# freewym/espresso

Measured on AMD Instinct MI355X. Metric: audio-hours/sec training (LibriSpeech Conformer-12 + CTC), higher is better.
Workload: dtype bf16; 1 GPU; LibriSpeech 960h Conformer-12 + CTC update step, <=26000 frames & <=24 utts per GPU, V=5004, on-GPU fbank+CMVN+SpecAugment, dropout 0.1, clip 2.0, Adam; parallelism=dp1

## Files before the change

### espresso_amd/csrc/flash_relpos.hip

```cpp
#include "flash_internal.h"

namespace {

typedef short bf16x4_t __attribute__((ext_vector_type(4)));
typedef const __attribute__((address_space(1))) void* gptr_t;
typedef __attribute__((address_space(3))) void* lptr_t;
typedef __attribute__((address_space(3))) bf16x4_t* lds_b4_t;

constexpr int DH = 64, TQ = 64, TK = 64;
constexpr int IMG = 64 * 128;
constexpr int BDP = 18;
constexpr int BNC = 80 * BDP * 4;
constexpr int OBP = 88;
constexpr int PP_OFF = 4 * IMG, BNC_OFF = 7 * IMG;
constexpr int LDS_BYTES = 7 * IMG + 4 * BNC;
constexpr int AUX_OFF = LDS_BYTES;
constexpr int LDS_BYTES_KV = LDS_BYTES + 1024;
constexpr float LOG2E = 1.4426950408889634f;

__device__ __forceinline__ int swz(int r) { return ((r >> 2) & 1) | (((r >> 1) & 1) << 1) | ((((r >> 2) ^ (r >> 3)) & 1) << 2); }

__device__ __forceinline__ int xcd_remap(int id, int total) {
  const int xcd = id & 7, q = total >> 3, r = total & 7;
  return (xcd < r ? xcd * (q + 1) : r * (q + 1) + (xcd - r) * q) + (id >> 3);
}
__device__ __forceinline__ f32x4_t mfma32(bf16x8_t a, bf16x8_t b, f32x4_t c) {
  return __builtin_amdgcn_mfma_f32_16x16x32_bf16(__builtin_bit_cast(__attribute__((ext_vector_type(8))) __bf16, a),
                                                 __builtin_bit_cast(__attribute__((ext_vector_type(8))) __bf16, b), c, 0, 0, 0);
}
__device__ __forceinline__ f32x4_t mfma16(bf16x4_t a, bf16x4_t b, f32x4_t c) {
  return __builtin_amdgcn_mfma_f32_16x16x16bf16_1k(a, b, c, 0, 0, 0);
}
__device__ __forceinline__ bf16x8_t cat(bf16x4_t lo, bf16x4_t hi) { return __builtin_shufflevector(lo, hi, 0, 1, 2, 3, 4, 5, 6, 7); }
__device__ __forceinline__ bf16x4_t pack4(float a, float b, float c, float d) {
  uint2 pk;
  pk.x = pack_bf2(a, b);
  pk.y = pack_bf2(c, d);
  return __builtin_bit_cast(bf16x4_t, pk);
}
__device__ __forceinline__ uint32_t lds_addr(const void* p) { return (uint32_t)(uintptr_t)p; }
template <int O0, int O1, int O2, int O3>
__device__ __forceinline__ void trr16(const uint32_t (&ad)[4], uint2 (&o)[16]) {
  asm volatile(
      "ds_read_b64_tr_b16 %0, %16 offset:%20\n\tds_read_b64_tr_b16 %1, %16 offset:%21\n\t"
      "ds_read_b64_tr_b16 %2, %16 offset:%22\n\tds_read_b64_tr_b16 %3, %16 offset:%23\n\t"
      "ds_read_b64_tr_b16 %4, %17 offset:%20\n\tds_read_b64_tr_b16 %5, %17 offset:%21\n\t"
      "ds_read_b64_tr_b16 %6, %17 offset:%22\n\tds_read_b64_tr_b16 %7, %17 offset:%23\n\t"
      "ds_read_b64_tr_b16 %8, %18 offset:%20\n\tds_read_b64_tr_b16 %9, %18 offset:%21\n\t"
      "ds_read_b64_tr_b16 %10, %18 offset:%22\n\tds_read_b64_tr_b16 %11, %18 offset:%23\n\t"
      "ds_read_b64_tr_b16 %12, %19 offset:%20\n\tds_read_b64_tr_b16 %13, %19 offset:%21\n\t"
      "ds_read_b64_tr_b16 %14, %19 offset:%22\n\tds_read_b64_tr_b16 %15, %19 offset:%23\n\t"
      "s_waitcnt lgkmcnt(0)"
      : "=&v"(o[0]), "=&v"(o[1]), "=&v"(o[2]), "=&v"(o[3]), "=&v"(o[4]), "=&v"(o[5]), "=&v"(o[6]), "=&v"(o[7]), "=&v"(o[8]),
        "=&v"(o[9]), "=&v"(o[10]), "=&v"(o[11]), "=&v"(o[12]), "=&v"(o[13]), "=&v"(o[14]), "=&v"(o[15])
      : "v"(ad[0]), "v"(ad[1]), "v"(ad[2]), "v"(ad[3]), "i"(O0), "i"(O1), "i"(O2), "i"(O3)
      : "memory");
}
template <int O0, int O1, int O2, int O3>
__device__ __forceinline__ void trr8(const uint32_t (&ad)[2], uint2 (&o)[8]) {
  asm volatile(
      "ds_read_b64_tr_b16 %0, %8 offset:%10\n\tds_read_b64_tr_b16 %1, %8 offset:%11\n\t"
      "ds_read_b64_tr_b16 %2, %8 offset:%12\n\tds_read_b64_tr_b16 %3, %8 offset:%13\n\t"
      "ds_read_b64_tr_b16 %4, %9 offset:%10\n\tds_read_b64_tr_b16 %5, %9 offset:%11\n\t"
      "ds_read_b64_tr_b16 %6, %9 offset:%12\n\tds_read_b64_tr_b16 %7, %9 offset:%13\n\t"
      "s_waitcnt lgkmcnt(0)"
      : "=&v"(o[0]), "=&v"(o[1]), "=&v"(o[2]), "=&v"(o[3]), "=&v"(o[4]), "=&v"(o[5]), "=&v"(o[6]), "=&v"(o[7])
      : "v"(ad[0]), "v"(ad[1]), "i"(O0), "i"(O1), "i"(O2), "i"(O3)
      : "memory");
}
__device__ __forceinline__ void trr20(const uint32_t (&ad)[20], uint2 (&o)[20]) {
  asm volatile(
      "ds_read_b64_tr_b16 %0, %20\n\tds_read_b64_tr_b16 %1, %21\n\tds_read_b64_tr_b16 %2, %22\n\tds_read_b64_tr_b16 %3, %23\n\t"
      "ds_read_b64_tr_b16 %4, %24\n\tds_read_b64_tr_b16 %5, %25\n\tds_read_b64_tr_b16 %6, %26\n\tds_read_b64_tr_b16 %7, %27\n\t"
      "ds_read_b64_tr_b16 %8, %28\n\tds_read_b64_tr_b16 %9, %29\n\tds_read_b64_tr_b16 %10, %30\n\tds_read_b64_tr_b16 %11, %31\n\t"
      "ds_read_b64_tr_b16 %12, %32\n\tds_read_b64_tr_b16 %13, %33\n\tds_read_b64_tr_b16 %14, %34\n\tds_read_b64_tr_b16 %15, %35\n\t"
      "ds_read_b64_tr_b16 %16, %36\n\tds_read_b64_tr_b16 %17, %37\n\tds_read_b64_tr_b16 %18, %38\n\tds_read_b64_tr_b16 %19, %39\n\t"
      "s_waitcnt lgkmcnt(0)"
      : "=&v"(o[0]), "=&v"(o[1]), "=&v"(o[2]), "=&v"(o[3]), "=&v"(o[4]), "=&v"(o[5]), "=&v"(o[6]), "=&v"(o[7]), "=&v"(o[8]),
        "=&v"(o[9]), "=&v"(o[10]), "=&v"(o[11]), "=&v"(o[12]), "=&v"(o[13]), "=&v"(o[14]), "=&v"(o[15]), "=&v"(o[16]),
        "=&v"(o[17]), "=&v"(o[18]), "=&v"(o[19])
      : "v"(ad[0]), "v"(ad[1]), "v"(ad[2]), "v"(ad[3]), "v"(ad[4]), "v"(ad[5]), "v"(ad[6]), "v"(ad[7]), "v"(ad[8]), "v"(ad[9]),
        "v"(ad[10]), "v"(ad[11]), "v"(ad[12]), "v"(ad[13]), "v"(ad[14]), "v"(ad[15]), "v"(ad[16]), "v"(ad[17]), "v"(ad[18]),
        "v"(ad[19])
      : "memory");
}
__device__ __forceinline__ uint2 lds_u2(const char* p) {
  const float* f = reinterpret_cast<const float*>(p);
  return make_uint2(__float_as_uint(f[0]), __float_as_uint(f[1]));
}
__device__ __forceinline__ bf16x8_t cat2(uint2 lo, uint2 hi) {
  return __builtin_bit_cast(bf16x8_t, make_uint4(lo.x, lo.y, hi.x, hi.y));
}
__device__ __forceinline__ void tr_image(const char* img, const uint32_t (&tro)[4], bf16x8_t (&f)[8]) {
  const uint32_t b = lds_addr(img);
  const uint32_t ad[4] = {b + tro[0], b + tro[1], b + tro[2], b + tro[3]};
  uint2 o[16];
  trr16<0, 2048, 4096, 6144>(ad, o);
#pragma unroll
  for (int dt = 0; dt < 4; ++dt) {
    f[dt * 2 + 0] = cat2(o[dt * 4 + 0], o[dt * 4 + 1]);
// ... 216 lines not shown
#pragma unroll
        for (int r = 0; r < 4; ++r)
          if (j0 + jt * 16 + g4 * 4 + r >= kl) acc_s[jt][r] = -INFINITY;
    }
    float tmax = fmaxf(fmaxf(acc_s[0][0], acc_s[0][1]), fmaxf(acc_s[0][2], acc_s[0][3]));
#pragma unroll
    for (int jt = 1; jt < 4; ++jt) tmax = fmaxf(tmax, fmaxf(fmaxf(acc_s[jt][0], acc_s[jt][1]), fmaxf(acc_s[jt][2], acc_s[jt][3])));
    tmax = fmaxf(tmax, __shfl_xor(tmax, 16, 64));
    tmax = fmaxf(tmax, __shfl_xor(tmax, 32, 64));
    const float m_new = fmaxf(m_run, tmax);
    const float msc = (m_new == -INFINITY) ? 0.f : m_new * LOG2E;
    const float alpha = fexp2(m_run * LOG2E - msc);
    float psum = 0.f;
#pragma unroll
    for (int jt = 0; jt < 4; ++jt)
#pragma unroll
      for (int r = 0; r < 4; ++r) {
        const float p = fexp2(fmaf(acc_s[jt][r], LOG2E, -msc));
        psum += p;
        acc_s[jt][r] = DROP ? fand(p, keep_mask(piece, ksh + jt * 4 + r)) : p;
      }
    l_run = l_run * alpha + psum;
    m_run = m_new;
#pragma unroll
    for (int dt = 0; dt < 4; ++dt)
#pragma unroll
      for (int r = 0; r < 4; ++r) acc_o[dt][r] *= alpha;

    {
      bf16x8_t vf[8];
      tr_image(sV, L.tro, vf);
#pragma unroll
      for (int kb = 0; kb < 2; ++kb) {
        const bf16x8_t pb = cat(pack4(acc_s[2 * kb][0], acc_s[2 * kb][1], acc_s[2 * kb][2], acc_s[2 * kb][3]),
                                pack4(acc_s[2 * kb + 1][0], acc_s[2 * kb + 1][1], acc_s[2 * kb + 1][2], acc_s[2 * kb + 1][3]));
#pragma unroll
        for (int dt = 0; dt < 4; ++dt) acc_o[dt] = mfma32(vf[dt * 2 + kb], pb, acc_o[dt]);
      }
    }
    slot_lo = slot_hi;
  }

  l_run += __shfl_xor(l_run, 16, 64);
  l_run += __shfl_xor(l_run, 32, 64);
  if (i < T) {
    const float inv = (DROP ? a.inv_keep : 1.f) / l_run;
    bf16_t* o = a.out + ((long)b * T + i) * a.ldo + h * DH;
#pragma unroll
    for (int dt = 0; dt < 4; ++dt) {
      uint2 pk;
      pk.x = pack_bf2(acc_o[dt][0] * inv, acc_o[dt][1] * inv);
      pk.y = pack_bf2(acc_o[dt][2] * inv, acc_o[dt][3] * inv);
      *reinterpret_cast<uint2*>(o + dt * 16 + g4 * 4) = pk;
    }
    if (a.lse && g4 == 0) a.lse[(long)z * T + i] = m_run + __logf(l_run);
  }
}

template <bool DROP, bool WANT_PD>
__device__ __forceinline__ void softmax_bwd_tile(f32x4_t (&acc_s)[4], const f32x4_t (&acc_dp)[4], bf16x4_t (&dsb)[4], bf16x4_t (&pdb)[4],
                                                 float lse2, float Di, float inv_keep, uint32_t piece, int ksh, int jrel_end, int g4) {
#pragma unroll
  for (int jt = 0; jt < 4; ++jt) {
    float ds[4], pd[4];
#pragma unroll
    for (int r = 0; r < 4; ++r) {
      float p = fexp2(fmaf(acc_s[jt][r], LOG2E, -lse2));
      if (jrel_end < 64 && jt * 16 + g4 * 4 + r >= jrel_end) p = 0.f;
      float dp = acc_dp[jt][r];
      if (DROP) {
        const uint32_t m = keep_mask(piece, ksh + jt * 4 + r);
        dp = fand(dp * inv_keep, m);
        if (WANT_PD) pd[r] = fand(p * inv_keep, m);
      } else if (WANT_PD) {
        pd[r] = p;
      }
      ds[r] = p * (dp - Di);
    }
    dsb[jt] = pack4(ds[0], ds[1], ds[2], ds[3]);
    if (WANT_PD) pdb[jt] = pack4(pd[0], pd[1], pd[2], pd[3]);
  }
}

template <bool DROP>
__global__ __launch_bounds__(256, 2) void rp_bwd_q_kernel(const FlashBwdArgs a) {
  __shared__ __attribute__((aligned(16))) char lds[LDS_BYTES];
  const LaneK L = lane_consts();
  const int lane = L.lane, w = L.w, li = L.li, g4 = L.g4;
  const int vid = xcd_remap(blockIdx.x, gridDim.x);
  const int z = vid / a.nq, qt = vid % a.nq;
  const int h = z / a.B, b = z % a.B;
  const int T = a.T;
  const int i0 = qt * TQ;
  const int i = i0 + 16 * w + li;
  const int kl = a.klen ? min(a.klen[b], T) : T;
  const int nt = (kl + TK - 1) / TK;
  const int nkt = (T + TK - 1) / TK;

  bf16x8_t qu[2], qv[2], dO[2];
  float Di = 0.f;
  {
    const int ic = min(i, T - 1);
    const long oq = ((long)b * T + ic) * a.ldq + h * DH + g4 * 8;
    const long oo = ((long)b * T + ic) * a.ldo + h * DH + g4 * 8;
#pragma unroll
    for (int ks = 0; ks < 2; ++ks) {
      qu[ks] = __builtin_bit_cast(bf16x8_t, *reinterpret_cast<const uint4*>(a.qu + oq + ks * 32));
      qv[ks] = __builtin_bit_cast(bf16x8_t, *reinterpret_cast<const uint4*>(a.qv + oq + ks * 32));
      const uint4 g = *reinterpret_cast<const uint4*>(a.dout + oo + ks * 32);
      const uint4 o = *reinterpret_cast<const uint4*>(a.out + oo + ks * 32);
      dO[ks] = __builtin_bit_cast(bf16x8_t, g);
      const uint32_t wg[4] = {g.x, g.y, g.z, g.w}, wo[4] = {o.x, o.y, o.z, o.w};
#pragma unroll
      for (int e = 0; e < 4; ++e)
        Di += __uint_as_float(wg[e] << 16) * __uint_as_float(wo[e] << 16) +
              __uint_as_float(wg[e] & 0xffff0000u) * __uint_as_float(wo[e] & 0xffff0000u);
    }
  }
  Di += __shfl_xor(Di, 16, 64);
  Di += __shfl_xor(Di, 32, 64);
  const float lse2 = (i < T) ? a.lse[(long)z * T + i] * LOG2E : INFINITY;
  if (i < T && g4 == 0 && a.D) a.D[(long)z * T + i] = Di;

  f32x4_t acc_t1[4], acc_t2[4];
#pragma unroll
  for (int dt = 0; dt < 4; ++dt) {
    acc_t1[dt] = (f32x4_t){0.f, 0.f, 0.f, 0.f};
    acc_t2[dt] = (f32x4_t){0.f, 0.f, 0.f, 0.f};
  }
  const bf16_t* Kb = a.k + (long)b * T * a.ldkv + h * DH;
  const bf16_t* Vb = a.v + (long)b * T * a.ldkv + h * DH;
  const bf16_t* PPb = a.pp + h * DH;
  const int R = 2 * T - 1;
  const ImgSrc srcK = img_src(Kb, a.ldkv, T - 1, w, lane), srcV = img_src(Vb, a.ldkv, T - 1, w, lane);
  const ImgSrc srcP = img_src(PPb, a.ldpp, R - 1, w, lane);
  const int pbase = (T - 1) - (i0 + TQ - 1);
  float* bd = reinterpret_cast<float*>(lds + BNC_OFF + w * BNC);
  bf16_t* ob = reinterpret_cast<bf16_t*>(bd);
  const uint32_t* bitp = DROP ? reinterpret_cast<const uint32_t*>(a.bits) + (((long)z * nkt) * (nkt * 64) + i) * 2 + (g4 >> 1) : nullptr;
  const long bit_step = (long)nkt * 64 * 2;
  const int ksh = (g4 & 1) * 16;
  uint2 mlo, mhi;
  {
    uint32_t m[4], n[4];
#pragma unroll
    for (int e = 0; e < 4; ++e) {
      m[e] = (4 * g4 + e >= 15 - li) ? 0xffffu : 0u;
      n[e] = (64 + 4 * g4 + e <= 78 - li) ? 0xffffu : 0u;
    }
    mlo = make_uint2(m[0] | (m[1] << 16), m[2] | (m[3] << 16));
    mhi = make_uint2(n[0] | (n[1] << 16), n[2] | (n[3] << 16));
  }
  const int ob_w = li * (OBP - 1) + 15 + g4 * 4;
  const char* ob_rd = reinterpret_cast<const char*>(ob) + li * (OBP * 2) + g4 * 8;

  uint32_t piece = 0, piece_next = 0;
  int jcov = 0;
  uint32_t dbd_pk[8];
  int dbd_j0 = -1;
  auto store_dbd = [&]() {
    const int j = dbd_j0 + lane;
    if (dbd_j0 >= 0 && j < T) {
      const int row_w = i0 + 16 * w, nrow = T - row_w;
      bf16_t* dp = a.dBD + ((long)z * T + row_w) * a.ld_bd + (T - 1 - row_w) + j;
      if (nrow >= 16) {
#pragma unroll
        for (int iw = 0; iw < 16; ++iw) dp[(long)iw * (a.ld_bd - 1)] = (bf16_t)(dbd_pk[iw >> 1] >> (16 * (iw & 1)));
      } else {
#pragma unroll
        for (int iw = 0; iw < 16; ++iw)
          if (iw < nrow) dp[(long)iw * (a.ld_bd - 1)] = (bf16_t)(dbd_pk[iw >> 1] >> (16 * (iw & 1)));
      }
    }
  };
  if (nt > 0) {
    issue_img(lds, srcK, 0, w, lane);
    issue_img(lds + IMG, srcV, 0, w, lane);
    issue_img(lds + PP_OFF, srcP, pbase, w, lane);
    issue_img(lds + PP_OFF + IMG, srcP, pbase + 64, w, lane);
    if (DROP) piece_next = bitp[0];
  }
  int slot_lo = 0;
  for (int t = 0; t < nt; ++t) {
    const int j0 = t * TK;
    jcov = min(T, j0 + TK);
    asm volatile("s_waitcnt vmcnt(0)" ::: "memory");
    __builtin_amdgcn_s_barrier();
    store_dbd();
    const int slot_hi = slot_lo == 2 ? 0 : slot_lo + 1;
    const int slot_nx = slot_hi == 2 ? 0 : slot_hi + 1;
    if (DROP) {
      piece = piece_next;
      asm volatile("" : "+v"(piece));
    }
    if (t + 1 < nt) {
      if (DROP) piece_next = bitp[(long)(t + 1) * bit_step];
      char* st = lds + ((t + 1) & 1) * 2 * IMG;
      issue_img(st, srcK, j0 + TK, w, lane);
      issue_img(st + IMG, srcV, j0 + TK, w, lane);
      issue_img(lds + PP_OFF + slot_nx * IMG, srcP, pbase + 64 * (t + 2), w, lane);
    }
    const char* sK = lds + (t & 1) * 2 * IMG;
    const char* sV = sK + IMG;
// ... 55 lines not shown
      for (int q16 = 0; q16 < 5; ++q16) {
        const int qq = q16 - w + 3;
        const uint32_t pbk = lds_addr(((qq >> 2) ? blk_hi : blk_lo) + (qq & 3) * 2048);
#pragma unroll
        for (int dt = 0; dt < 4; ++dt) ad[q16 * 4 + dt] = pbk + L.tro[dt];
      }
      trr20(ad, pf);
#pragma unroll
      for (int cb = 0; cb < 2; ++cb) {
        uint2 blo = lds_u2(ob_rd + cb * 64);
        const uint2 bhi = lds_u2(ob_rd + cb * 64 + 32);
        if (cb == 0) {
          blo.x &= mlo.x;
          blo.y &= mlo.y;
        }
        const bf16x8_t db = cat2(blo, bhi);
#pragma unroll
        for (int dt = 0; dt < 4; ++dt) acc_t2[dt] = mfma32(cat2(pf[(2 * cb) * 4 + dt], pf[(2 * cb + 1) * 4 + dt]), db, acc_t2[dt]);
      }
      uint2 bl = lds_u2(ob_rd + 128);
      bl.x &= mhi.x;
      bl.y &= mhi.y;
#pragma unroll
      for (int dt = 0; dt < 4; ++dt)
        acc_t2[dt] = mfma16(__builtin_bit_cast(bf16x4_t, pf[16 + dt]), __builtin_bit_cast(bf16x4_t, bl), acc_t2[dt]);
    }
    {
      const bf16_t* bs = ob + 15 + lane;
#pragma unroll
      for (int k = 0; k < 8; ++k)
        dbd_pk[k] = (uint32_t)bs[(2 * k) * (OBP - 1)] | ((uint32_t)bs[(2 * k + 1) * (OBP - 1)] << 16);
      dbd_j0 = j0;
    }
    wave_lds_sync();
    slot_lo = slot_hi;
  }
  store_dbd();

  if (i < T) {
    bf16_t* o1 = a.t1 + ((long)b * T + i) * a.ldt + h * DH;
    bf16_t* o2 = a.t2 + ((long)b * T + i) * a.ldt + h * DH;
#pragma unroll
    for (int dt = 0; dt < 4; ++dt) {
      uint2 pk;
      pk.x = pack_bf2(acc_t1[dt][0] * a.scaling, acc_t1[dt][1] * a.scaling);
      pk.y = pack_bf2(acc_t1[dt][2] * a.scaling, acc_t1[dt][3] * a.scaling);
      *reinterpret_cast<uint2*>(o1 + dt * 16 + g4 * 4) = pk;
      pk.x = pack_bf2(acc_t2[dt][0] * a.scaling, acc_t2[dt][1] * a.scaling);
      pk.y = pack_bf2(acc_t2[dt][2] * a.scaling, acc_t2[dt][3] * a.scaling);
      *reinterpret_cast<uint2*>(o2 + dt * 16 + g4 * 4) = pk;
    }
    if (a.dq) {
      bf16_t* oq = a.dq + ((long)b * T + i) * a.lddq + h * DH;
#pragma unroll
      for (int dt = 0; dt < 4; ++dt) {
        uint2 pk;
        pk.x = pack_bf2((acc_t1[dt][0] + acc_t2[dt][0]) * a.scaling, (acc_t1[dt][1] + acc_t2[dt][1]) * a.scaling);
        pk.y = pack_bf2((acc_t1[dt][2] + acc_t2[dt][2]) * a.scaling, (acc_t1[dt][3] + acc_t2[dt][3]) * a.scaling);
        *reinterpret_cast<uint2*>(oq + dt * 16 + g4 * 4) = pk;
      }
    }
  }
  if (!a.dbd_prezeroed) {
    for (int iw = 0; iw < 16; ++iw) {
      const int row = i0 + 16 * w + iw;
      if (row >= T) break;
      const int lo = T - 1 - row, hi = lo + jcov;
      bf16_t* dr = a.dBD + ((long)z * T + row) * a.ld_bd;
      for (int c = lane; c * 8 < a.ld_bd; c += 64) {
        const int e0 = c * 8;
        if (e0 + 8 <= lo || e0 >= hi) {
          *reinterpret_cast<uint4*>(dr + e0) = make_uint4(0, 0, 0, 0);
        } else if (e0 < lo || e0 + 8 > hi) {
#pragma unroll
          for (int e = 0; e < 8; ++e)
            if (e0 + e < lo || e0 + e >= hi) dr[e0 + e] = 0;
        }
      }
    }
  }
}

template <bool DROP>
__global__ __launch_bounds__(256, 2) void rp_bwd_kv_kernel(const FlashBwdArgs a) {
  __shared__ __attribute__((aligned(16))) char lds[LDS_BYTES_KV];
  const LaneK L = lane_consts();
  const int lane = L.lane, w = L.w, li = L.li, g4 = L.g4;
  const int vid = xcd_remap(blockIdx.x, gridDim.x);
  const int z = vid / a.nk, kt = vid % a.nk;
  const int h = z / a.B, b = z % a.B;
  const int T = a.T;
  const int j0 = kt * TK;
  const int kl = a.klen ? min(a.klen[b], T) : T;
  const int nq = (j0 < kl) ? a.nq : 0;
  const int nkt = a.nk;

  bf16x8_t kf[4][2], vf[4][2];
#pragma unroll
  for (int jt = 0; jt < 4; ++jt) {
    const int j = min(j0 + jt * 16 + li, T - 1);
    const long o = ((long)b * T + j) * a.ldkv + h * DH + g4 * 8;
#pragma unroll
    for (int ks = 0; ks < 2; ++ks) {
      kf[jt][ks] = __builtin_bit_cast(bf16x8_t, *reinterpret_cast<const uint4*>(a.k + o + ks * 32));
      vf[jt][ks] = __builtin_bit_cast(bf16x8_t, *reinterpret_cast<const uint4*>(a.v + o + ks * 32));
    }
  }
  f32x4_t acc_dk[4], acc_dv[4];
#pragma unroll
  for (int dt = 0; dt < 4; ++dt) {
    acc_dk[dt] = (f32x4_t){0.f, 0.f, 0.f, 0.f};
    acc_dv[dt] = (f32x4_t){0.f, 0.f, 0.f, 0.f};
  }
  const bf16_t* Qub = a.qu + (long)b * T * a.ldq + h * DH;
  const bf16_t* Qvb = a.qv + (long)b * T * a.ldq + h * DH;
  const bf16_t* dOb = a.dout + (long)b * T * a.ldo + h * DH;
  const bf16_t* PPb = a.pp + h * DH;
  const int R = 2 * T - 1;
  const ImgSrc srcQ = img_src(Qub, a.ldq, T - 1, w, lane), srcG = img_src(dOb, a.ldo, T - 1, w, lane);
  const ImgSrc srcP = img_src(PPb, a.ldpp, R - 1, w, lane);
  const int pb0 = (T - 1) - (TQ - 1) + j0;
  float* bd = reinterpret_cast<float*>(lds + BNC_OFF + w * BNC);
  char* exw = lds + BNC_OFF + w * BNC;
  const uint32_t exo = li * 128 + ((((g4 >> 1) ^ swz(li))) << 4) + (g4 & 1) * 8;
  uint32_t exr[2], trk[2];
#pragma unroll
  for (int hh = 0; hh < 2; ++hh) {
    const int rl = 8 * (g4 & 1) + 4 * hh + (li >> 2);
    exr[hh] = (g4 >> 1) * BNC + rl * 128 + (((2 * w + ((li & 3) >> 1)) ^ swz(rl)) << 4) + (li & 1) * 8;
    const int rr = 8 * g4 + 4 * hh + (li >> 2);
    trk[hh] = rr * 128 + ((((li & 3) >> 1) ^ swz(rr)) << 4) + (li & 1) * 8;
  }
  const char* exbase = lds + BNC_OFF;
  const uint32_t* bitp = DROP ? reinterpret_cast<const uint32_t*>(a.bits) + (((long)z * nkt + kt) * (nkt * 64) + 16 * w + li) * 2 + (g4 >> 1) : nullptr;
  const int ksh = (g4 & 1) * 16;

  bf16x8_t qv[2], qv_next[2];
  uint32_t piece_next = 0;
  auto row_loads = [&](int i0, int stage) {
    const int i = i0 + 16 * w + li;
    const int ic = min(i, T - 1);
    const long o = (long)ic * a.ldq + g4 * 8;
    qv_next[0] = __builtin_bit_cast(bf16x8_t, *reinterpret_cast<const uint4*>(Qvb + o));
    qv_next[1] = __builtin_bit_cast(bf16x8_t, *reinterpret_cast<const uint4*>(Qvb + o + 32));
    if (DROP) piece_next = bitp[(long)i0 * 2];
    if (w < 2) {
      const float* src = (w == 0 ? a.lse : a.D) + (long)z * T + min(i0 + lane, T - 1);
      __builtin_amdgcn_global_load_lds((gptr_t)src, (lptr_t)(lds + AUX_OFF + stage * 512 + w * 256), 4, 0, 0);
    }
  };
  if (nq > 0) {
    issue_img(lds, srcQ, 0, w, lane);
    issue_img(lds + IMG, srcG, 0, w, lane);
    issue_img(lds + PP_OFF, srcP, pb0, w, lane);
    issue_img(lds + PP_OFF + 2 * IMG, srcP, pb0 + 64, w, lane);
    row_loads(0, 0);
  }
  int slot_lo = 0;
  for (int it = 0; it < nq; ++it) {
    const int i0 = it * TQ;
    asm volatile("s_waitcnt vmcnt(0)" ::: "memory");
    __builtin_amdgcn_s_barrier();
    const int slot_hi = slot_lo == 0 ? 2 : slot_lo - 1;
    const int slot_nx = slot_lo == 2 ? 0 : slot_lo + 1;
    qv[0] = qv_next[0];
    qv[1] = qv_next[1];
    const float* aux = reinterpret_cast<const float*>(lds + AUX_OFF + (it & 1) * 512) + 16 * w + li;
    const float lse_raw = aux[0], Di = aux[64];
    uint32_t piece = piece_next;
    {
      uint4 q0 = __builtin_bit_cast(uint4, qv[0]), q1 = __builtin_bit_cast(uint4, qv[1]);
      asm volatile("" : "+v"(q0.x), "+v"(q0.y), "+v"(q0.z), "+v"(q0.w), "+v"(q1.x), "+v"(q1.y), "+v"(q1.z), "+v"(q1.w), "+v"(piece));
      qv[0] = __builtin_bit_cast(bf16x8_t, q0);
      qv[1] = __builtin_bit_cast(bf16x8_t, q1);
    }
    const float lse2 = (i0 + 16 * w + li < T) ? lse_raw * LOG2E : INFINITY;
    if (it + 1 < nq) {
      row_loads(i0 + TQ, (it + 1) & 1);
      char* st = lds + ((it + 1) & 1) * 2 * IMG;
      issue_img(st, srcQ, i0 + TQ, w, lane);
      issue_img(st + IMG, srcG, i0 + TQ, w, lane);
      issue_img(lds + PP_OFF + slot_nx * IMG, srcP, pb0 - 64 * (it + 1), w, lane);
    }
    const char* sQ = lds + (it & 1) * 2 * IMG;
    const char* sG = sQ + IMG;
    bf16x8_t qu[2], dO[2];
#pragma unroll
    for (int ks = 0; ks < 2; ++ks) {
      qu[ks] = ldf(sQ + w * 2048 + L.offk[ks]);
      dO[ks] = ldf(sG + w * 2048 + L.offk[ks]);
    }
    f32x4_t acc_s[4], acc_dp[4];
#pragma unroll
    for (int jt = 0; jt < 4; ++jt) {
      acc_s[jt] = (f32x4_t){0.f, 0.f, 0.f, 0.f};
      acc_dp[jt] = (f32x4_t){0.f, 0.f, 0.f, 0.f};
    }
#pragma unroll
    for (int ks = 0; ks < 2; ++ks)
#pragma unroll
      for (int jt = 0; jt < 4; ++jt) {
        acc_s[jt] = mfma32(kf[jt][ks], qu[ks], acc_s[jt]);
        acc_dp[jt] = mfma32(vf[jt][ks], dO[ks], acc_dp[jt]);
      }
    add_band(acc_s, qv, lds + PP_OFF + slot_lo * IMG, lds + PP_OFF + slot_hi * IMG, bd, L);
    bf16x4_t dsb[4], pdb[4];
    softmax_bwd_tile<DROP, true>(acc_s, acc_dp, dsb, pdb, lse2, Di, a.inv_keep, piece, ksh, kl - j0, g4);
    wave_lds_sync();
#pragma unroll
    for (int jt = 0; jt < 4; ++jt) {
      *reinterpret_cast<bf16x4_t*>(exw + (exo ^ (jt << 5))) = dsb[jt];
      *reinterpret_cast<bf16x4_t*>(exw + 2048 + (exo ^ (jt << 5))) = pdb[jt];
    }
    asm volatile("s_waitcnt lgkmcnt(0)" ::: "memory");
    __builtin_amdgcn_s_barrier();
    {
      const uint32_t eb = lds_addr(exbase);
      const uint32_t ead[2] = {eb + exr[0], eb + exr[1]};
      uint2 bx[8];
      trr8<0, 2048, 2 * BNC, 2 * BNC + 2048>(ead, bx);
      const uint32_t qb = lds_addr(sQ);
#pragma unroll
      for (int half = 0; half < 2; ++half) {
        const int d0 = half * 2;
        const uint32_t aad[4] = {qb + (trk[0] ^ (uint32_t)(d0 << 5)), qb + (trk[1] ^ (uint32_t)(d0 << 5)),
                                 qb + (trk[0] ^ (uint32_t)((d0 + 1) << 5)), qb + (trk[1] ^ (uint32_t)((d0 + 1) << 5))};
        uint2 ax[16];
        trr16<0, 4096, IMG, IMG + 4096>(aad, ax);
#pragma unroll
        for (int dd = 0; dd < 2; ++dd)
#pragma unroll
          for (int ks2 = 0; ks2 < 2; ++ks2) {
            const bf16x8_t aq = cat2(ax[(dd * 2 + 0) * 4 + ks2], ax[(dd * 2 + 1) * 4 + ks2]);
            const bf16x8_t ag = cat2(ax[(dd * 2 + 0) * 4 + 2 + ks2], ax[(dd * 2 + 1) * 4 + 2 + ks2]);
            acc_dk[d0 + dd] = mfma32(aq, cat2(bx[0 * 4 + 2 * ks2], bx[1 * 4 + 2 * ks2]), acc_dk[d0 + dd]);
            acc_dv[d0 + dd] = mfma32(ag, cat2(bx[0 * 4 + 2 * ks2 + 1], bx[1 * 4 + 2 * ks2 + 1]), acc_dv[d0 + dd]);
          }
      }
    }
    slot_lo = slot_nx;
  }
  const int j = j0 + 16 * w + li;
  if (j < T) {
    bf16_t* ok = a.dk + ((long)b * T + j) * a.lddkv + h * DH;
    bf16_t* ov = a.dv + ((long)b * T + j) * a.lddkv + h * DH;
#pragma unroll
    for (int dt = 0; dt < 4; ++dt) {
      uint2 pk;
      pk.x = pack_bf2(acc_dk[dt][0], acc_dk[dt][1]);
      pk.y = pack_bf2(acc_dk[dt][2], acc_dk[dt][3]);
      *reinterpret_cast<uint2*>(ok + dt * 16 + g4 * 4) = pk;
      pk.x = pack_bf2(acc_dv[dt][0], acc_dv[dt][1]);
      pk.y = pack_bf2(acc_dv[dt][2], acc_dv[dt][3]);
      *reinterpret_cast<uint2*>(ov + dt * 16 + g4 * 4) = pk;
    }
  }
}

}

static int g_rp_on = 1;
extern "C" int ea_set_flash_relpos(int on) {
  const int prev = g_rp_on;
  g_rp_on = on ? 1 : 0;
  return prev;
}
bool ea_rp_eligible(bool relpos, int T, int S, int causal, uint32_t thr, const void* bits) {
  return g_rp_on && relpos && T == S && !(causal & 1) && (thr == 0 || bits != nullptr);
}

int ea_rp_keep_bits(uint16_t* bits, int H, int B, int T, uint64_t seed, uint32_t thr, hipStream_t stream) {
  const int nkt = (T + TK - 1) / TK;
  const long n = (long)H * B * nkt * (nkt * 64) * 4;
  constexpr long cap = 256;
  long blocks = (n + 255) / 256;
  if (blocks > cap) blocks = cap;
  hipLaunchKernelGGL(keep_bits_kernel, dim3((unsigned)blocks), dim3(256), 0, stream, bits, seed, thr, H * B, T, nkt);
  return EA_CHECK_LAUNCH();
}

int ea_rp_fwd(const FlashFwdArgs& a, hipStream_t stream) {
  const dim3 grid((unsigned)(a.nq * a.H * a.B));
  if (a.thr) hipLaunchKernelGGL(rp_fwd_kernel<true>, grid, dim3(256), 0, stream, a);
  else hipLaunchKernelGGL(rp_fwd_kernel<false>, grid, dim3(256), 0, stream, a);
  return EA_CHECK_LAUNCH();
}

int ea_rp_bwd(const FlashBwdArgs& a, hipStream_t stream) {
  const dim3 gq((unsigned)(a.nq * a.H * a.B)), gk((unsigned)(a.nk * a.H * a.B));
  if (a.thr) {
    hipLaunchKernelGGL(rp_bwd_q_kernel<true>, gq, dim3(256), 0, stream, a);
    hipLaunchKernelGGL(rp_bwd_kv_kernel<true>, gk, dim3(256), 0, stream, a);
  } else {
    hipLaunchKernelGGL(rp_bwd_q_kernel<false>, gq, dim3(256), 0, stream, a);
    hipLaunchKernelGGL(rp_bwd_kv_kernel<false>, gk, dim3(256), 0, stream, a);
  }
  return EA_CHECK_LAUNCH();
}
```

### include/espresso_amd.h

```cpp
#ifndef ESPRESSO_AMD_H
#define ESPRESSO_AMD_H

#include <stdint.h>

#ifdef __cplusplus
extern "C" {
#endif

typedef struct ihipStream_t* ea_stream_t;

int ea_version(void);

enum { EA_ACT_NONE = 0, EA_ACT_RELU = 1, EA_ACT_SILU = 2 };

typedef struct EaGemmParams {
  const void* A;
  const void* B;
  void* C;
  void* C2;
  const float* bias;
  const void* resid;
  const void* aux;
  int M, N, K, batch, zdiv;
  int a_kstrided, b_kstrided, c_f32, accumulate, resid_f32, act;
// ... 23 lines not shown
int ea_set_gemm_w8(int mode);
int ea_gemm_profile_enable(int on);
long ea_gemm_profile_read(double* total_ms, double* total_flops);
int ea_gemm_profile_bytes(double* total_bytes);
long ea_gemm_profile_dump(const char* path);

#define EA_WGRAD_MAX 16
typedef struct EaWgradProblem {
  const void* dy;
  const void* x;
  float* dW;
  float* dbias;
  int M, N, K;
  long ld_dy, ld_x, ldw;
} EaWgradProblem;
typedef struct EaWgradGroup {
  int count;
  EaWgradProblem p[EA_WGRAD_MAX];
} EaWgradGroup;
int ea_wgrad_group(const EaWgradGroup* group, ea_stream_t stream);
int ea_set_wgrad_transposing_reads(int on);
int ea_set_wgrad_w8(int mode);

int ea_layernorm_fwd(const void* x, const float* gamma, const float* beta, void* y, float* mean, float* rstd,
                     int M, int C, float eps, const uint8_t* row_zero, uint64_t drop_seed, uint32_t drop_thr,
                     float drop_scale, ea_stream_t stream);
int ea_layernorm_fwd_f32out(const void* x, const float* gamma, const float* beta, float* y, float* mean, float* rstd,
                            int M, int C, float eps, const uint8_t* row_zero, uint64_t drop_seed, uint32_t drop_thr,
                            float drop_scale, ea_stream_t stream);
int ea_layernorm_bwd_f32dy(const void* x, const float* dy, const float* gamma, const float* mean, const float* rstd,
                           void* dx, float* dgamma, float* dbeta, int M, int C, const uint8_t* row_zero,
                           uint64_t drop_seed, uint32_t drop_thr, float drop_scale, const void* dx_add,
                           void* workspace, ea_stream_t stream);
long ea_layernorm_bwd_workspace_bytes(int M, int C);
int ea_layernorm_bwd(const void* x, const void* dy, const float* gamma, const float* mean, const float* rstd,
                     void* dx, float* dgamma, float* dbeta, int M, int C, const uint8_t* row_zero,
                     uint64_t drop_seed, uint32_t drop_thr, float drop_scale, const void* dx_add,
                     void* workspace, ea_stream_t stream);
int ea_layernorm_bwd_dx(const void* x, const void* dy, const float* gamma, const float* mean, const float* rstd, void* dx,
                        float* dgamma, float* dbeta, int M, int C, const uint8_t* row_zero, uint64_t drop_seed,
                        uint32_t drop_thr, float drop_scale, const void* dx_add, void* workspace, ea_stream_t stream);
int ea_layernorm_param_reduce(const void* workspace, float* dgamma, float* dbeta, int M, int C, ea_stream_t stream);
#define EA_LNRED_MAX 8
typedef struct EaLnReduceItem { const void* workspace; float* dgamma; float* dbeta; int M, C; } EaLnReduceItem;
typedef struct EaLnReduceGroup { int count; EaLnReduceItem item[EA_LNRED_MAX]; } EaLnReduceGroup;
int ea_layernorm_param_reduce_group(const EaLnReduceGroup* group, ea_stream_t stream);
int ea_layernorm_bwd_dx2(const void* x, const void* dy, const float* gamma, const float* mean, const float* rstd, void* dx,
                         float* dgamma, float* dbeta, int M, int C, const void* dx_add, void* workspace, void* out2, float a2,
                         uint64_t seed2, uint32_t thr2, float scale2, ea_stream_t stream);
int ea_layernorm_fwd2(const void* x, const float* g1, const float* b1, void* y1, float* mean1, float* rstd1, const float* g2,
                      const float* b2, void* y2, float* mean2, float* rstd2, int M, int C, float eps, ea_stream_t stream);
int ea_layernorm_bwd2_dx(const void* x1, const void* dy1, const float* gamma1, const float* mean1, const float* rstd1,
                         const void* dx_add, void* ws1, const void* x2, const float* gamma2, const float* mean2, const float* rstd2,
                         void* ws2, void* dx, int M, int C, void* out2, float a2, uint64_t seed2, uint32_t thr2, float scale2,
                         ea_stream_t stream);

int ea_cast_f32_to_bf16(const float* src, void* dst, long n, ea_stream_t stream);
int ea_transpose_bf16_batch(const void* const* src, void* const* dst, const int* rows, const int* cols, int n, ea_stream_t stream);
int ea_audio_probe(const char* path, long* num_samples, int* sample_rate, int* channels, int* bits);
long ea_audio_read_i16(const char* path, int16_t* dst, long capacity, int* sample_rate);
int ea_audio_verify(const char* path);
int ea_audio_read_batch_i16(const char* const* paths, int n, int16_t* dst, const long* offsets, int num_threads, long* lengths,
                            int* sample_rates);

int ea_cast_f32_to_bf16_rows(const float* src, long ld_src, void* dst, long ld_dst, long M, int N, ea_stream_t stream);
int ea_cast_bf16_to_f32(const void* src, float* dst, long n, ea_stream_t stream);
int ea_scale_dropout_bf16(const void* x, const void* y, void* out, long n, float a, float b, uint64_t seed,
                          uint32_t thr, float inv_keep, ea_stream_t stream);
int ea_colsum_bf16(const void* X, float* out, int M, int N, long ld, ea_stream_t stream);
int ea_embedding_fwd(const int* tokens, const int* positions, const float* W, const float* pos_table, void* out, int M,
                     int C, float scale, ea_stream_t stream);
int ea_embedding_bwd(const int* tokens, const void* dy, float* dW, int M, int C, float scale, int pad_idx,
                     ea_stream_t stream);
int ea_zero_rows_bf16(void* x, const uint8_t* row_zero, int M, int C, ea_stream_t stream);

int ea_flash_attention_supported(int dh, int T, int S, int relpos);
int ea_flash_attention_fwd(const void* qu, const void* qv, long ldq, const void* k, const void* v, long ldkv,
                           const void* pp, long ldpp, const int* key_len, void* out, long ldo, float* lse, int H, int B,
                           int T, int S, int dh, int causal, uint64_t drop_seed, uint32_t drop_thr, float drop_scale,
                           void* keep_bits, ea_stream_t stream);
long ea_flash_keep_bits_bytes(int H, int B, int T);
int ea_set_flash_relpos(int on);
int ea_flash_keep_bits(void* keep_bits, int H, int B, int T, uint64_t drop_seed, uint32_t drop_thr, ea_stream_t stream);
int ea_flash_attention_bwd(const void* qu, const void* qv, long ldq, const void* k, const void* v, long ldkv,
                           const void* pp, long ldpp, const int* key_len, const void* out, const void* dout, long ldo,
                           const float* lse, float* D, void* t1, void* t2, long ldt, void* dBD, int ld_bd, void* dk,
                           void* dv, long lddkv, int H, int B, int T, int S, int dh, int causal, float scaling,
                           uint64_t drop_seed, uint32_t drop_thr, float drop_scale, const void* keep_bits,
                           void* dq, long lddq, ea_stream_t stream);

int ea_relpos_q_prep(const void* qkv, long ldq, const float* u, const float* v, void* qu, void* qv, int M,
                     int C, float scaling, ea_stream_t stream);
int ea_relpos_softmax_fwd(const float* ac, const float* bd, const int* key_len, const float* attn_mask, void* P,
                          void* Pd, int H, int B, int T, int S, int ld_ac, int ld_bd, int ld_p, int causal,
                          uint64_t drop_seed, uint32_t drop_thr, float drop_scale, ea_stream_t stream);
int ea_relpos_softmax_bwd(const void* P, const float* dPd, void* dAC, void* dBD, int H, int B, int T, int S,
                          int ld_p, int ld_dp, int ld_bd, uint64_t drop_seed, uint32_t drop_thr,
                          float drop_scale, ea_stream_t stream);
int ea_add2_strided_bf16(const void* a, long lda, const void* b, long ldb, void* out, long ldo, int M, int C,
                         ea_stream_t stream);

int ea_glu_dwconv_fwd(const void* Y, const float* w, void* U, void* Z, double* stats, int B, int T, int C, int KW,
                      ea_stream_t stream);
int ea_bn_finalize(const double* stats, float* mean_rstd, float* running_mean, float* running_var, int C, float n,
                   float eps, float momentum, ea_stream_t stream);
int ea_bn_from_running(const float* running_mean, const float* running_var, float* mean_rstd, int C, float eps,
                       ea_stream_t stream);
int ea_bn_act_fwd(const void* Z, const float* mean_rstd, const float* gamma, const float* beta, void* H, long M,
                  int C, int act, ea_stream_t stream);
int ea_bn_act_bwd(const void* Z, const void* dH, const float* mean_rstd, const float* gamma, const float* beta,
                  float* red, void* dZ, float* dgamma, float* dbeta, long M, int C, int act, int training,
                  ea_stream_t stream);
long ea_dwconv_wgrad_workspace_bytes(int B, int T, int C, int KW);
int ea_glu_dwconv_bwd(const void* dZ, const void* Y, const void* U, const float* w, void* dY, float* dw,
                      void* wgrad_ws, int B, int T, int C, int KW, ea_stream_t stream);
int ea_dwconv_bwd_weight(const void* dZ, const void* U, float* dw, void* wgrad_ws, int B, int T, int C, int KW, ea_stream_t stream);
int ea_glu_dwconv_causal_fwd(const void* Y, const float* w, void* U, void* Z, double* stats, int B, int T, int C, int KW,
                             ea_stream_t stream);
int ea_glu_dwconv_causal_bwd(const void* dZ, const void* Y, const void* U, const float* w, void* dY, float* dw,
                             void* wgrad_ws, int B, int T, int C, int KW, ea_stream_t stream);
int ea_dwconv_causal_bwd_weight(const void* dZ, const void* U, float* dw, void* wgrad_ws, int B, int T, int C, int KW,
                                ea_stream_t stream);
int ea_bn_act_fwd_train(const void* Z, const double* stats, float* mean_rstd, float* running_mean, float* running_var,
                        const float* gamma, const float* beta, void* H, long M, int C, int act, float n, float eps,
                        float momentum, double* zero_next, int zero_n, ea_stream_t stream);
int ea_bn_act_bwd_fused(const void* Z, const void* dH, const float* mean_rstd, const float* gamma, const float* beta,
                        float* red, void* dZ, float* dgamma, float* dbeta, long M, int C, int act, int training,
                        float* zero_next, int zero_n, ea_stream_t stream);
int ea_bn_param_grad(const float* red, float* dgamma, float* dbeta, int C, ea_stream_t stream);
int ea_conv1_bn_bwd(const float* X, const void* Z, const void* dH, const float* mean_rstd, const float* gamma, const float* beta,
                    float* red, float* dgamma, float* dbeta, float* dW, float* dbias, int B, int T, int F, int CO, int sy, int sx,
                    int act, int training, ea_stream_t stream);

int ea_conv1_fwd(const float* X, const float* W, const float* bias, void* Z, double* stats, int B, int T, int F,
                 int CO, int sy, int sx, ea_stream_t stream);
int ea_conv1_wgrad(const float* X, const void* dZ, float* dW, float* dbias, int B, int T, int F, int CO, int sy,
                   int sx, ea_stream_t stream);
int ea_conv3x3_fwd(const void* X, const void* W, const float* bias, void* Z, double* stats, int B, int T, int F, int Cin,
                   int Cout, int sy, int sx, ea_stream_t stream);
int ea_conv3x3_dgrad(const void* dZ, const void* Wd, void* dX, int B, int T, int F, int Cin, int Cout, int sy, int sx,
                     ea_stream_t stream);
long ea_conv3x3_wgrad_workspace_bytes(int B, int T, int F, int Cin, int Cout, int sy, int sx);
int ea_conv3x3_wgrad(const void* X, const void* dZ, float* dW, void* workspace, int B, int T, int F, int Cin, int Cout, int sy,
                     int sx, ea_stream_t stream);
int ea_conv3x3_wgrad_param_layout(const void* X, const void* dZ, float* dW, void* workspace, int B, int T, int F, int Cin, int Cout,
                                  int sy, int sx, ea_stream_t stream);
int ea_im2col3x3(const void* A, void* col, int B, int T, int F, int C, int sy, int sx, ea_stream_t stream);
int ea_col2im3x3(const void* dcol, void* dA, int B, int T, int F, int C, int sy, int sx, ea_stream_t stream);
int ea_colstats_bf16(const void* X, double* stats, long M, int C, ea_stream_t stream);

int ea_log_softmax_f32(const float* in, long ld_in, float* out, long M, int V, ea_stream_t stream);
int ea_log_softmax_bf16(const void* in, long ld_in, float* out, long M, int V, ea_stream_t stream);
long ea_ctc_workspace_bytes(int B, int T, int Lmax);
int ea_ctc_loss(const float* lprobs, const int* targets, const int* in_len, const int* tgt_len, float* nll,
                void* workspace, int B, int T, int V, int Lmax, int blank, ea_stream_t stream);
int ea_ctc_grad(const float* lprobs, const void* workspace, const float* nll, const int* targets,
                const int* in_len, const int* tgt_len, void* dlogits, long ld_out, int dlogits_bf16, int B, int T,
                int V, int Lmax, int blank, float grad_scale, const float* grad_scale_dev, int zero_infinity,
                ea_stream_t stream);
int ea_ctc_greedy_decode(const void* x, long ld, int x_bf16, const int* in_len, int* best, float* bestv, int* tokens,
                         int* align, int* out_len, float* score, int B, int T, int V, int blank, int pad,
                         ea_stream_t stream);
long ea_ctc_prefix_beam_workspace_bytes(int B, int T, int beam);
int ea_ctc_prefix_beam_step(const void* x, long ld, int x_bf16, const int* in_len, void* workspace, const float* lm_rows,
                            long ld_lm, int* lm_parent, int* lm_token, void* lm_keep, int B, int T, int V, int beam, int K,
                            int blank, float lm_weight, float ins_bonus, int t0, int t1, ea_stream_t stream);
// ... 369 lines not shown
```

Before: 5.343 audio-hours/sec.

## Fuse relpos attention backward dq and dkv kernels into one launch

Merges the query-side and key/value-side relative-position flash attention backward kernels into a single grid. Blocks below the padded query count run the dq body and the rest run the dkv body, so both can execute concurrently and the launch gap disappears. To drop the dkv kernel's dependence on the D vector written by the dq kernel, the dkv body now recomputes D per row from dO and the prefetched output rows instead of loading it. This adds extra global loads and dot products in the dkv loop and uses the larger LDS footprint for every block. Older launch orders stay selectable through a new setter.

```diff
diff --git a/espresso_amd/csrc/flash_relpos.hip b/espresso_amd/csrc/flash_relpos.hip
--- a/espresso_amd/csrc/flash_relpos.hip
+++ b/espresso_amd/csrc/flash_relpos.hip
@@ -15,7 +15,8 @@
 constexpr int PP_OFF = 4 * IMG, BNC_OFF = 7 * IMG;
 constexpr int LDS_BYTES = 7 * IMG + 4 * BNC;
 constexpr int AUX_OFF = LDS_BYTES;
-constexpr int LDS_BYTES_KV = LDS_BYTES + 1024;
+constexpr int LDS_BYTES_KV = LDS_BYTES + 512;
+constexpr int LDS_BYTES_BWD = LDS_BYTES_KV > LDS_BYTES ? LDS_BYTES_KV : LDS_BYTES;
 constexpr float LOG2E = 1.4426950408889634f;
 
 __device__ __forceinline__ int swz(int r) { return ((r >> 2) & 1) | (((r >> 1) & 1) << 1) | ((((r >> 2) ^ (r >> 3)) & 1) << 2); }
@@ -398,12 +399,26 @@
   }
 }
 
+__device__ __forceinline__ float row_dot(const uint4 (&g)[2], const uint4 (&o)[2]) {
+  float Di = 0.f;
+#pragma unroll
+  for (int ks = 0; ks < 2; ++ks) {
+    const uint32_t wg[4] = {g[ks].x, g[ks].y, g[ks].z, g[ks].w}, wo[4] = {o[ks].x, o[ks].y, o[ks].z, o[ks].w};
+#pragma unroll
+    for (int e = 0; e < 4; ++e)
+      Di += __uint_as_float(wg[e] << 16) * __uint_as_float(wo[e] << 16) +
+            __uint_as_float(wg[e] & 0xffff0000u) * __uint_as_float(wo[e] & 0xffff0000u);
+  }
+  Di += __shfl_xor(Di, 16, 64);
+  Di += __shfl_xor(Di, 32, 64);
+  return Di;
+}
+
 template <bool DROP>
-__global__ __launch_bounds__(256, 2) void rp_bwd_q_kernel(const FlashBwdArgs a) {
-  __shared__ __attribute__((aligned(16))) char lds[LDS_BYTES];
+__device__ __forceinline__ void rp_bwd_q_body(const FlashBwdArgs& a, char* lds, int wg, int total) {
   const LaneK L = lane_consts();
   const int lane = L.lane, w = L.w, li = L.li, g4 = L.g4;
-  const int vid = xcd_remap(blockIdx.x, gridDim.x);
+  const int vid = xcd_remap(wg, total);
   const int z = vid / a.nq, qt = vid % a.nq;
   const int h = z / a.B, b = z % a.B;
   const int T = a.T;
@@ -414,27 +429,22 @@
   const int nkt = (T + TK - 1) / TK;
 
   bf16x8_t qu[2], qv[2], dO[2];
-  float Di = 0.f;
+  float Di;
   {
     const int ic = min(i, T - 1);
     const long oq = ((long)b * T + ic) * a.ldq + h * DH + g4 * 8;
     const long oo = ((long)b * T + ic) * a.ldo + h * DH + g4 * 8;
+    uint4 g[2], o[2];
 #pragma unroll
     for (int ks = 0; ks < 2; ++ks) {
       qu[ks] = __builtin_bit_cast(bf16x8_t, *reinterpret_cast<const uint4*>(a.qu + oq + ks * 32));
       qv[ks] = __builtin_bit_cast(bf16x8_t, *reinterpret_cast<const uint4*>(a.qv + oq + ks * 32));
-      const uint4 g = *reinterpret_cast<const uint4*>(a.dout + oo + ks * 32);
-      const uint4 o = *reinterpret_cast<const uint4*>(a.out + oo + ks * 32);
-      dO[ks] = __builtin_bit_cast(bf16x8_t, g);
-      const uint32_t wg[4] = {g.x, g.y, g.z, g.w}, wo[4] = {o.x, o.y, o.z, o.w};
-#pragma unroll
-      for (int e = 0; e < 4; ++e)
-        Di += __uint_as_float(wg[e] << 16) * __uint_as_float(wo[e] << 16) +
-              __uint_as_float(wg[e] & 0xffff0000u) * __uint_as_float(wo[e] & 0xffff0000u);
-    }
-  }
-  Di += __shfl_xor(Di, 16, 64);
-  Di += __shfl_xor(Di, 32, 64);
+      g[ks] = *reinterpret_cast<const uint4*>(a.dout + oo + ks * 32);
+      o[ks] = *reinterpret_cast<const uint4*>(a.out + oo + ks * 32);
+      dO[ks] = __builtin_bit_cast(bf16x8_t, g[ks]);
+    }
+    Di = row_dot(g, o);
+  }
   const float lse2 = (i < T) ? a.lse[(long)z * T + i] * LOG2E : INFINITY;
   if (i < T && g4 == 0 && a.D) a.D[(long)z * T + i] = Di;
 
@@ -656,11 +666,10 @@
 }
 
 template <bool DROP>
-__global__ __launch_bounds__(256, 2) void rp_bwd_kv_kernel(const FlashBwdArgs a) {
-  __shared__ __attribute__((aligned(16))) char lds[LDS_BYTES_KV];
+__device__ __forceinline__ void rp_bwd_kv_body(const FlashBwdArgs& a, char* lds, int wg, int total) {
   const LaneK L = lane_consts();
   const int lane = L.lane, w = L.w, li = L.li, g4 = L.g4;
-  const int vid = xcd_remap(blockIdx.x, gridDim.x);
+  const int vid = xcd_remap(wg, total);
   const int z = vid / a.nk, kt = vid % a.nk;
   const int h = z / a.B, b = z % a.B;
   const int T = a.T;
@@ -689,6 +698,7 @@
   const bf16_t* Qub = a.qu + (long)b * T * a.ldq + h * DH;
   const bf16_t* Qvb = a.qv + (long)b * T * a.ldq + h * DH;
   const bf16_t* dOb = a.dout + (long)b * T * a.ldo + h * DH;
+  const bf16_t* Ob = a.out + (long)b * T * a.ldo + h * DH;
   const bf16_t* PPb = a.pp + h * DH;
   const int R = 2 * T - 1;
   const ImgSrc srcQ = img_src(Qub, a.ldq, T - 1, w, lane), srcG = img_src(dOb, a.ldo, T - 1, w, lane);
@@ -710,6 +720,7 @@
   const int ksh = (g4 & 1) * 16;
 
   bf16x8_t qv[2], qv_next[2];
+  uint4 og[2];
   uint32_t piece_next = 0;
   auto row_loads = [&](int i0, int stage) {
     const int i = i0 + 16 * w + li;
@@ -718,10 +729,15 @@
     qv_next[0] = __builtin_bit_cast(bf16x8_t, *reinterpret_cast<const uint4*>(Qvb + o));
     qv_next[1] = __builtin_bit_cast(bf16x8_t, *reinterpret_cast<const uint4*>(Qvb + o + 32));
     if (DROP) piece_next = bitp[(long)i0 * 2];
-    if (w < 2) {
-      const float* src = (w == 0 ? a.lse : a.D) + (long)z * T + min(i0 + lane, T - 1);
-      __builtin_amdgcn_global_load_lds((gptr_t)src, (lptr_t)(lds + AUX_OFF + stage * 512 + w * 256), 4, 0, 0);
-    }
+    if (w == 0) {
+      const float* src = a.lse + (long)z * T + min(i0 + lane, T - 1);
+      __builtin_amdgcn_global_load_lds((gptr_t)src, (lptr_t)(lds + AUX_OFF + stage * 256), 4, 0, 0);
+    }
+  };
+  auto out_loads = [&](int i0) {
+    const long oo = (long)min(i0 + 16 * w + li, T - 1) * a.ldo + g4 * 8;
+    og[0] = *reinterpret_cast<const uint4*>(Ob + oo);
+    og[1] = *reinterpret_cast<const uint4*>(Ob + oo + 32);
   };
   if (nq > 0) {
     issue_img(lds, srcQ, 0, w, lane);
@@ -729,6 +745,7 @@
     issue_img(lds + PP_OFF, srcP, pb0, w, lane);
     issue_img(lds + PP_OFF + 2 * IMG, srcP, pb0 + 64, w, lane);
     row_loads(0, 0);
+    out_loads(0);
   }
   int slot_lo = 0;
   for (int it = 0; it < nq; ++it) {
@@ -739,8 +756,7 @@
     const int slot_nx = slot_lo == 2 ? 0 : slot_lo + 1;
     qv[0] = qv_next[0];
     qv[1] = qv_next[1];
-    const float* aux = reinterpret_cast<const float*>(lds + AUX_OFF + (it & 1) * 512) + 16 * w + li;
-    const float lse_raw = aux[0], Di = aux[64];
+    const float lse_raw = reinterpret_cast<const float*>(lds + AUX_OFF + (it & 1) * 256)[16 * w + li];
     uint32_t piece = piece_next;
     {
       uint4 q0 = __builtin_bit_cast(uint4, qv[0]), q1 = __builtin_bit_cast(uint4, qv[1]);
@@ -764,6 +780,15 @@
       qu[ks] = ldf(sQ + w * 2048 + L.offk[ks]);
       dO[ks] = ldf(sG + w * 2048 + L.offk[ks]);
     }
+    const uint4 gg[2] = {__builtin_bit_cast(uint4, dO[0]), __builtin_bit_cast(uint4, dO[1])};
+    float Di;
+    {
+      typedef float f32x2_t __attribute__((ext_vector_type(2)));
+      const float d = row_dot(gg, og);
+      f32x2_t d2 = {d, d};
+      asm volatile("" : "+v"(d2));
+      Di = d2.x;
+    }
     f32x4_t acc_s[4], acc_dp[4];
 #pragma unroll
     for (int jt = 0; jt < 4; ++jt) {
@@ -788,6 +813,7 @@
     }
     asm volatile("s_waitcnt lgkmcnt(0)" ::: "memory");
     __builtin_amdgcn_s_barrier();
+    if (it + 1 < nq) out_loads(i0 + TQ);
     {
       const uint32_t eb = lds_addr(exbase);
       const uint32_t ead[2] = {eb + exr[0], eb + exr[1]};
@@ -831,6 +857,27 @@
   }
 }
 
+template <bool DROP>
+__global__ __launch_bounds__(256, 2) void rp_bwd_kernel(const FlashBwdArgs a) {
+  __shared__ __attribute__((aligned(16))) char lds[LDS_BYTES_BWD];
+  const int gq = a.nq * a.H * a.B, gk = a.nk * a.H * a.B;
+  const int gq8 = (gq + 7) & ~7;
+  const int id = (int)blockIdx.x;
+  if (id >= gq8) rp_bwd_kv_body<DROP>(a, lds, id - gq8, gk);
+  else if (id < gq) rp_bwd_q_body<DROP>(a, lds, id, gq);
+}
+
+template <bool DROP>
+__global__ __launch_bounds__(256, 2) void rp_bwd_q_kernel(const FlashBwdArgs a) {
+  __shared__ __attribute__((aligned(16))) char lds[LDS_BYTES];
+  rp_bwd_q_body<DROP>(a, lds, (int)blockIdx.x, (int)gridDim.x);
+}
+template <bool DROP>
+__global__ __launch_bounds__(256, 2) void rp_bwd_kv_kernel(const FlashBwdArgs a) {
+  __shared__ __attribute__((aligned(16))) char lds[LDS_BYTES_KV];
+  rp_bwd_kv_body<DROP>(a, lds, (int)blockIdx.x, (int)gridDim.x);
+}
+
 }
 
 static int g_rp_on = 1;
@@ -860,14 +907,28 @@
   return EA_CHECK_LAUNCH();
 }
 
+static int g_rp_bwd_launches = 1;
+extern "C" int ea_set_flash_relpos_bwd_launches(int n) {
+  const int prev = g_rp_bwd_launches;
+  if (n == 1 || n == 2 || n == -2) g_rp_bwd_launches = n;
+  return prev;
+}
+
+template <bool DROP>
+static void rp_bwd_launch(const FlashBwdArgs& a, hipStream_t stream) {
+  const unsigned gq = (unsigned)(a.nq * a.H * a.B), gk = (unsigned)(a.nk * a.H * a.B);
+  const int mode = g_rp_bwd_launches;
+  if (mode == 1) {
+    hipLaunchKernelGGL(rp_bwd_kernel<DROP>, dim3(((gq + 7) & ~7u) + gk), dim3(256), 0, stream, a);
+    return;
+  }
+  if (mode == 2) hipLaunchKernelGGL(rp_bwd_q_kernel<DROP>, dim3(gq), dim3(256), 0, stream, a);
+  hipLaunchKernelGGL(rp_bwd_kv_kernel<DROP>, dim3(gk), dim3(256), 0, stream, a);
+  if (mode == -2) hipLaunchKernelGGL(rp_bwd_q_kernel<DROP>, dim3(gq), dim3(256), 0, stream, a);
+}
+
 int ea_rp_bwd(const FlashBwdArgs& a, hipStream_t stream) {
-  const dim3 gq((unsigned)(a.nq * a.H * a.B)), gk((unsigned)(a.nk * a.H * a.B));
-  if (a.thr) {
-    hipLaunchKernelGGL(rp_bwd_q_kernel<true>, gq, dim3(256), 0, stream, a);
-    hipLaunchKernelGGL(rp_bwd_kv_kernel<true>, gk, dim3(256), 0, stream, a);
-  } else {
-    hipLaunchKernelGGL(rp_bwd_q_kernel<false>, gq, dim3(256), 0, stream, a);
-    hipLaunchKernelGGL(rp_bwd_kv_kernel<false>, gk, dim3(256), 0, stream, a);
-  }
+  if (a.thr) rp_bwd_launch<true>(a, stream);
+  else rp_bwd_launch<false>(a, stream);
   return EA_CHECK_LAUNCH();
 }
diff --git a/include/espresso_amd.h b/include/espresso_amd.h
--- a/include/espresso_amd.h
+++ b/include/espresso_amd.h
@@ -129,6 +129,7 @@
 long ea_flash_keep_bits_bytes(int H, int B, int T);
 int ea_set_flash_relpos(int on);
 int ea_flash_keep_bits(void* keep_bits, int H, int B, int T, uint64_t drop_seed, uint32_t drop_thr, ea_stream_t stream);
+int ea_set_flash_relpos_bwd_launches(int n);
 int ea_flash_attention_bwd(const void* qu, const void* qv, long ldq, const void* k, const void* v, long ldkv,
                            const void* pp, long ldpp, const int* key_len, const void* out, const void* dout, long ldo,
                            const float* lse, float* D, void* t1, void* t2, long ldt, void* dBD, int ld_bd, void* dk,
```

Result: no change. 5.360 audio-hours/sec, median of 6 (+0.3%).
